# josebeo2016/SCL-Deepfake-audio-detection

Measured on AMD Instinct MI355X. Metric: train-step utterances/sec (64000-sample clips), higher is better.
Workload: dtype bf16

## Files before the change

### scl-deepfake-audio-detection_amd/csrc/gemm_w8.hip

```cpp
#include "gemm_common.h"
#include "gemm_w8_epi.h"

using namespace sclg;

__device__ unsigned long long scl_gemm_stamps[4096 * 8];

namespace {

__device__ __forceinline__ void w8_stamp(const GemmK& d, int slot, int lane, int wave) {
    if ((d.flags & SCL_GEMM_STAMPS) && wave == 0 && lane == 0 && blockIdx.x < 4096 && blockIdx.z == 0) {
        scl_gemm_stamps[blockIdx.x * 8 + 2 * slot] = __builtin_amdgcn_s_memrealtime();
        scl_gemm_stamps[blockIdx.x * 8 + 2 * slot + 1] = __builtin_amdgcn_s_memtime();
    }
}

constexpr int W8_BN = 256;
constexpr int W8_OPB = 2 * TILE_BYTES;
constexpr int W8_NA = 3, W8_NB = 2;
constexpr int W8_LDS = (W8_NA + W8_NB) * W8_OPB;

struct W8K {
    __amdgpu_buffer_rsrc_t rsrc;
    unsigned voff[4];
    __device__ __forceinline__ void init(const OpK& o, const char* base, int row0, int rowlimit, int lane, int wave) {
// ... 330 lines not shown
#define W8S_B_ISSUE(j) if ((j) < 2) { lb.issue1(tB, wave, soffB, live2b, 2 * (j)); lb.issue1(tB, wave, soffB, live2b, 2 * (j) + 1); }
#define W8S_Q_SECOND(j, R0, R1)                                                                                              \
        RD::template go<R0, R1, false>(fa0, fb0, a_nxt, tBn, ab, nbk, 0, lane);                                              \
        __builtin_amdgcn_sched_barrier(0);                                                                                   \
        _Pragma("unroll") for (int i = 0; i < RBW; ++i)                                                                      \
            acc[i][j] = __builtin_amdgcn_mfma_f32_16x16x32_bf16(fb1[j], fa1[i], acc[i][j], 0, 0, 0);                         \
        __builtin_amdgcn_sched_barrier(0);                                                                                   \
        W8S_B_ISSUE(j)                                                                                                       \
        __builtin_amdgcn_sched_barrier(0);
        W8S_Q_SECOND(0, 0, RQ0) W8S_Q_SECOND(1, RQ0, RQ1) W8S_Q_SECOND(2, RQ1, RQ2) W8S_Q_SECOND(3, RQ2, NRD)
#undef W8S_Q_SECOND
#undef W8S_B_ISSUE
        char* t = a_cur; a_cur = a_nxt; a_nxt = a_fill; a_fill = t;
    }
    asm volatile("s_waitcnt vmcnt(0)" ::: "memory");
    asm volatile("s_waitcnt lgkmcnt(0)" ::: "memory");
    __builtin_amdgcn_s_barrier();
    w8_stamp(d, 2, lane, wave);
    {
        const long long cbase = z1 * d.c_bs1 + z2 * d.c_bs2 + (long long)ksplit * d.c_split_stride;
        const float* bias = (d.flags & SCL_GEMM_HAS_BIAS) ? d.bias + z2 * d.bias_bs2 : nullptr;
        char* wlds = smem + wave * 16384;
        char* wextra = smem + 8 * 16384 + wave * 4096;
        float* cs0 = d.colsum ? d.colsum + ((long long)(m0 / d.tile_m) * 4 + (wave >> 2) * 2) * d.N : nullptr;
        if constexpr (RBW >= 4) {
            f32x4 (&alo)[4][4] = *reinterpret_cast<f32x4 (*)[4][4]>(&acc[0]);
            w8_epilogue_pass<4, ((RBW < 8 && !AT) ? 0x1E : 0)>(d, alo, 4, wlds, wextra, m0 + ab * 16, n0 + wc * 64, mlimit, cbase, bias, lane, cs0);
        } else {
            f32x4 lo[4][4];
#pragma unroll
            for (int i = 0; i < 4; ++i)
#pragma unroll
                for (int j = 0; j < 4; ++j) lo[i][j] = (i < RBW) ? acc[(i < RBW) ? i : 0][j] : f32x4{0.f, 0.f, 0.f, 0.f};
            w8_epilogue_pass<4, ((RBW < 8 && !AT) ? 0x1E : 0)>(d, lo, RBW, wlds, wextra, m0 + ab * 16, n0 + wc * 64, mlimit, cbase, bias, lane, cs0);
        }
        if (RBW > 4) {
            f32x4 hi[4][4];
#pragma unroll
            for (int i = 0; i < 4; ++i)
#pragma unroll
                for (int j = 0; j < 4; ++j) hi[i][j] = (4 + i < RBW) ? acc[(4 + i < RBW) ? 4 + i : 0][j] : f32x4{0.f, 0.f, 0.f, 0.f};
            w8_epilogue_pass<4, ((RBW < 8 && !AT) ? 0x1E : 0)>(d, hi, RBW - 4, wlds, wextra, m0 + (ab + 4) * 16, n0 + wc * 64, mlimit, cbase, bias, lane, cs0 ? cs0 + d.N : nullptr);
        }
    }
    if (d.flags & SCL_GEMM_STAMPS) {
        asm volatile("s_waitcnt vmcnt(0)" ::: "memory");
        w8_stamp(d, 3, lane, wave);
    }
}

template <bool AT, bool BT, int RB0, int RB1, bool SEQ = false>
__device__ __forceinline__ void w8s_tile(const GemmK& d, char* smem, const int bid, const int nblk, const int bz) {
    const int tid = threadIdx.x, lane = tid & 63;
    const int wave = __builtin_amdgcn_readfirstlane(tid >> 6);
    const int wr = wave >> 2, wc = wave & 3;
    w8_stamp(d, 0, lane, wave);
#ifdef SCL_EXPERIMENTS
    if ((d.debug >> 8) && (bid & 1) && bid < 256 && bz == 0) {
        for (int i = 0; i < (d.debug >> 8); ++i) __builtin_amdgcn_s_sleep(127);
    }
#endif
    const int tiles_m = (d.M + d.tile_m - 1) / d.tile_m, tiles_n = (d.N + W8_BN - 1) / W8_BN;
    int tm, tn;
    tile_coords<SEQ>(bid, nblk, tiles_m, tiles_n, tm, tn, d.group_m);
    const int m0 = tm * d.tile_m, n0 = tn * W8_BN;
    const int mlimit = min(d.M, m0 + d.tile_m);
    int z = bz;
    const int ksplit = __builtin_amdgcn_readfirstlane(z % d.splitk); z /= d.splitk;
    const int z1 = __builtin_amdgcn_readfirstlane(z / d.nb2), z2 = z - z1 * d.nb2;
    const int nk_total = d.K / BK;
    const int nk_per = __builtin_amdgcn_readfirstlane((nk_total + d.splitk - 1) / d.splitk);
    const int kt0 = ksplit * nk_per;
    const int nk = max(0, min(nk_per, nk_total - kt0));
    const char* Ab = reinterpret_cast<const char*>(d.A.ptr) + z1 * d.A.bs1 + z2 * d.A.bs2;
    const char* Bb = reinterpret_cast<const char*>(d.B.ptr) + z1 * d.B.bs1 + z2 * d.B.bs2;

    typename W8Sel<AT>::type la;
    typename W8Sel<BT>::type lb;
    la.init(d.A, Ab, m0, mlimit, lane, wave);
    lb.init(d.B, Bb, n0, d.N, lane, wave);
    la.set_batched(false); lb.set_batched(false);
    const unsigned stepA = W8Sel<AT>::type::kstep(d.A), stepB = W8Sel<BT>::type::kstep(d.B);
    unsigned soffA = (unsigned)kt0 * stepA, soffB = (unsigned)kt0 * stepB;
    la.template issue2<0>(smem, wave, soffA, nk > 0); la.template issue2<2>(smem, wave, soffA, nk > 0);
    lb.template issue2<0>(smem + W8_NA * W8_OPB, wave, soffB, nk > 0); lb.template issue2<2>(smem + W8_NA * W8_OPB, wave, soffB, nk > 0);
    soffA += stepA; soffB += stepB;
    la.template issue2<0>(smem + W8_OPB, wave, soffA, nk > 1); la.template issue2<2>(smem + W8_OPB, wave, soffA, nk > 1);
    lb.template issue2<0>(smem + (W8_NA + 1) * W8_OPB, wave, soffB, nk > 1); lb.template issue2<2>(smem + (W8_NA + 1) * W8_OPB, wave, soffB, nk > 1);
    asm volatile("s_waitcnt vmcnt(8)" ::: "memory");
    w8_stamp(d, 1, lane, wave);
    __builtin_amdgcn_s_barrier();
    if (RB0 == RB1) {
        w8s_body<AT, BT, RB0>(d, smem, la, lb, nk, soffA, soffB, wr * RB0, m0, n0, mlimit, z1, z2, ksplit, lane, wave, wc);
    } else if (wr == 0) {
        w8s_body<AT, BT, RB0>(d, smem, la, lb, nk, soffA, soffB, 0, m0, n0, mlimit, z1, z2, ksplit, lane, wave, wc);
    } else {
        w8s_body<AT, BT, RB1>(d, smem, la, lb, nk, soffA, soffB, RB0, m0, n0, mlimit, z1, z2, ksplit, lane, wave, wc);
    }
}

template <bool AT, bool BT, int RB0, int RB1>
__global__ __launch_bounds__(512, 2) void scl_gemm_w8s_kernel(const GemmK d) {
    extern __shared__ __attribute__((aligned(16))) char smem[];
    w8s_tile<AT, BT, RB0, RB1>(d, smem, blockIdx.x, gridDim.x, blockIdx.z);
}

struct GemmGroupK {
    GemmK k[W8_GROUP_MAX];
    int first[W8_GROUP_MAX + 1];
    int tile0[W8_GROUP_MAX];
    int ntiles[W8_GROUP_MAX];
    int n;
    int xcd_major;
};
typedef const __attribute__((address_space(4))) GemmGroupK* W8GArg;
template <bool AT, bool BT, int RB0, int RB1>
__global__ __launch_bounds__(512, 2) void scl_gemm_w8s_group_kernel(const GemmGroupK g) {
    extern __shared__ __attribute__((aligned(16))) char smem[];
    W8GArg gp = (W8GArg)__builtin_amdgcn_kernarg_segment_ptr();
    const int total = g.first[W8_GROUP_MAX];
    const int x = blockIdx.x & 7, idx = blockIdx.x >> 3, q = total >> 3, r = total & 7;
#ifdef SCL_EXPERIMENTS
    const int pos = (g.xcd_major ? ((x < r ? x * (q + 1) : r * (q + 1) + (x - r) * q) + idx) : (int)blockIdx.x);
#else
    const int pos = (x < r ? x * (q + 1) : r * (q + 1) + (x - r) * q) + idx;
#endif
    int mem = 0;
#pragma unroll
    for (int i = 1; i < W8_GROUP_MAX; ++i) mem += (i < g.n && pos >= g.first[i]) ? 1 : 0;
    mem = __builtin_amdgcn_readfirstlane(mem);
    const int t = __builtin_amdgcn_readfirstlane(pos - gp->first[mem] + gp->tile0[mem]);
#ifdef SCL_EXPERIMENTS
    if (!g.xcd_major) { w8s_tile<AT, BT, RB0, RB1, false>(*(const GemmK*)&gp->k[mem], smem, t, gp->ntiles[mem], 0); return; }
#endif
    w8s_tile<AT, BT, RB0, RB1, true>(*(const GemmK*)&gp->k[mem], smem, t, gp->ntiles[mem], 0);
}

typedef const __attribute__((address_space(4))) GemmK* W8KArg;
__device__ __forceinline__ const GemmK* w8p_args(W8KArg p) {
    asm volatile("" : "+s"(p));
    return (const GemmK*)p;
}
__device__ __forceinline__ int w8p_lane() {
    int l = (int)__builtin_amdgcn_mbcnt_hi(~0u, __builtin_amdgcn_mbcnt_lo(~0u, 0u));
    asm volatile("" : "+v"(l));
    return l;
}
constexpr int W8_EPI_KEY = SCL_GEMM_C_F32 | SCL_GEMM_C2_F32 | SCL_GEMM_R_F32 | SCL_GEMM_HAS_BIAS | SCL_GEMM_HAS_C2 | SCL_GEMM_DROPOUT |
                           (0xF << SCL_GEMM_ACT_SHIFT) | (0xF << SCL_GEMM_RMODE_SHIFT) | (0xF << SCL_GEMM_RACT_SHIFT);
inline int w8p_epi_kind(int flags) {
    const int f = flags & W8_EPI_KEY, fb = f & ~SCL_GEMM_HAS_BIAS;
    if (fb == 0) return 1;
    if (f == (SCL_GEMM_HAS_BIAS | SCL_GEMM_HAS_C2 | (5 << SCL_GEMM_ACT_SHIFT))) return 2;
    if (fb == SCL_GEMM_C_F32) return 5;
    return 0;
}

template <bool AT, bool BT, int RBW, int EK>
__device__ __forceinline__ void w8p_body(W8KArg kp, char* smem, const int ab, const int lane, const int wave, const int wc) {
    typedef typename W8Sel<AT>::type LA;
    typedef typename W8Sel<BT>::type LB;
    typedef W8SRead<AT, BT, RBW> RD;
    constexpr int NRD = RBW + 4, OPA = AT ? 2 : 1, OPB = BT ? 2 : 1;
    constexpr int RQ0 = 4, RQ1 = 8, RQ2 = NRD;
    static_assert(RBW >= 6 && RBW <= 8, "w8p_body: 6 to 8 row blocks per wave");
    auto ops_upto = [](int n) constexpr { return (n > 0 ? OPB : 0) + (n > 1 ? (n - 1 < RBW ? n - 1 : RBW) * OPA : 0) + (n > RBW + 1 ? (n - RBW - 1) * OPB : 0); };
    const int nbk = wc * 4;
    char* const bimg = smem + W8_NA * W8_OPB;
    char *a_cur = smem, *a_nxt = smem + W8_OPB, *a_fill = smem + 2 * W8_OPB;
    LA la;
    LB lb;
    la.set_batched(false); lb.set_batched(false);
    int nk, tile_m, Mrows, group_m, tiles_m, tiles_n, m0, n0, mlimit;
    unsigned stepA, stepB;
    int v = blockIdx.x;
    {
        const GemmK* d0 = w8p_args(kp);
        nk = d0->K / BK;
        tile_m = d0->tile_m; Mrows = d0->M; group_m = d0->group_m;
        tiles_m = __builtin_amdgcn_readfirstlane((Mrows + tile_m - 1) / tile_m);
        tiles_n = (d0->N + W8_BN - 1) / W8_BN;
        if (v >= tiles_m * tiles_n) return;
        stepA = LA::kstep(d0->A); stepB = LB::kstep(d0->B);
        int tm, tn;
        tile_coords(v, tiles_m * tiles_n, tiles_m, tiles_n, tm, tn, group_m);
        m0 = tm * tile_m; n0 = tn * W8_BN; mlimit = min(Mrows, m0 + tile_m);
        la.init(d0->A, reinterpret_cast<const char*>(d0->A.ptr), m0, mlimit, lane, wave);
        lb.init(d0->B, reinterpret_cast<const char*>(d0->B.ptr), n0, d0->N, lane, wave);
    }
    const int ntiles = tiles_m * tiles_n, G = gridDim.x;
    la.template issue2<0>(a_cur, wave, 0u, true); la.template issue2<2>(a_cur, wave, 0u, true);
    lb.template issue2<0>(bimg, wave, 0u, true); lb.template issue2<2>(bimg, wave, 0u, true);
    la.template issue2<0>(a_nxt, wave, stepA, true); la.template issue2<2>(a_nxt, wave, stepA, true);
    lb.template issue2<0>(bimg + W8_OPB, wave, stepB, true); lb.template issue2<2>(bimg + W8_OPB, wave, stepB, true);
    asm volatile("s_waitcnt vmcnt(8)" ::: "memory");
    __builtin_amdgcn_s_barrier();
    int bpar = 0;
    unsigned soffA = stepA, soffB = stepB;
    int m0n = 0, n0n = 0, mlimn = 0;
    for (;;) {
        f32x4 acc[RBW][4];
#pragma unroll
        for (int i = 0; i < RBW; ++i)
#pragma unroll
            for (int j = 0; j < 4; ++j) acc[i][j] = f32x4{0.f, 0.f, 0.f, 0.f};
        bf16x8 fa0[RBW], fa1[RBW], fb0[4], fb1[4];
        const bool has_next = v + G < ntiles;
        lds_wait_upto(0);
        __builtin_amdgcn_sched_barrier(0);
        RD::template go<0, NRD, true>(fa0, fb0, a_cur, bimg + bpar * W8_OPB, ab, nbk, 0, lane);
        for (int kt = 0; kt < nk; ++kt) {
            char* tB = bimg + ((kt + bpar) & 1) * W8_OPB;
            const bool live2 = kt + 2 < nk || has_next;
            soffA += stepA; soffB += stepB;
            if (kt + 2 == nk) {
                soffA = 0u; soffB = 0u;
                if (has_next) {
                    int tm, tn;
                    tile_coords(v + G, ntiles, tiles_m, tiles_n, tm, tn, group_m);
                    m0n = tm * tile_m; n0n = tn * W8_BN; mlimn = min(Mrows, m0n + tile_m);
                    const GemmK* dh = w8p_args(kp);
                    const int ln = w8p_lane();
                    la.init(dh->A, reinterpret_cast<const char*>(dh->A.ptr), m0n, mlimn, ln, wave);
                    lb.init(dh->B, reinterpret_cast<const char*>(dh->B.ptr), n0n, dh->N, ln, wave);
                    lds_wait_upto(0);
                    __builtin_amdgcn_sched_barrier(0);
                }
            }
#define W8P_Q_FIRST(j, R0, R1)                                                                                               \
            RD::template go<R0, R1, false>(fa1, fb1, a_cur, tB, ab, nbk, 1, lane);                                           \
            __builtin_amdgcn_sched_barrier(0);                                                                               \
            lds_wait_upto((3 - (j)) * OPB + ops_upto(R1));                                                                   \
            __builtin_amdgcn_sched_barrier(0);                                                                               \
            _Pragma("unroll") for (int i = 0; i < RBW; ++i)                                                                  \
                acc[i][j] = __builtin_amdgcn_mfma_f32_16x16x32_bf16(fb0[j], fa0[i], acc[i][j], 0, 0, 0);                     \
            __builtin_amdgcn_sched_barrier(0);                                                                               \
            la.issue1(a_fill, wave, soffA, live2, j);                                                                        \
            __builtin_amdgcn_sched_barrier(0);
            W8P_Q_FIRST(0, 0, RQ0) W8P_Q_FIRST(1, RQ0, RQ1) W8P_Q_FIRST(2, RQ1, RQ2) W8P_Q_FIRST(3, RQ2, NRD)
#undef W8P_Q_FIRST
            lds_wait_upto(0);
            asm volatile("s_waitcnt vmcnt(4)" ::: "memory");
            __builtin_amdgcn_sched_barrier(0);
            __builtin_amdgcn_s_barrier();
            __builtin_amdgcn_sched_barrier(0);
            const char* tBn = bimg + (((kt + bpar) & 1) ^ 1) * W8_OPB;
#define W8P_B_ISSUE(j) if ((j) < 2) { lb.issue1(tB, wave, soffB, live2, 2 * (j)); lb.issue1(tB, wave, soffB, live2, 2 * (j) + 1); }
#define W8P_Q_SECOND(j, R0, R1)                                                                                              \
            RD::template go<R0, R1, false>(fa0, fb0, a_nxt, tBn, ab, nbk, 0, lane);                                          \
            __builtin_amdgcn_sched_barrier(0);                                                                               \
            _Pragma("unroll") for (int i = 0; i < RBW; ++i)                                                                  \
                acc[i][j] = __builtin_amdgcn_mfma_f32_16x16x32_bf16(fb1[j], fa1[i], acc[i][j], 0, 0, 0);                     \
            __builtin_amdgcn_sched_barrier(0);                                                                               \
            W8P_B_ISSUE(j)                                                                                                   \
            __builtin_amdgcn_sched_barrier(0);
            W8P_Q_SECOND(0, 0, RQ0) W8P_Q_SECOND(1, RQ0, RQ1) W8P_Q_SECOND(2, RQ1, RQ2) W8P_Q_SECOND(3, RQ2, NRD)
#undef W8P_Q_SECOND
#undef W8P_B_ISSUE
            char* t = a_cur; a_cur = a_nxt; a_nxt = a_fill; a_fill = t;
        }
        lds_wait_upto(0);
        __builtin_amdgcn_sched_barrier(0);
        {
            const GemmK& d = *w8p_args(kp);
            const int ln = w8p_lane();
            const float* bias = (EK == 2 || (d.flags & SCL_GEMM_HAS_BIAS)) ? d.bias : nullptr;
            char* wlds = a_fill + wave * 4096;
            float* cs0 = d.colsum ? d.colsum + ((long long)(m0 / tile_m) * 4 + (wave >> 2) * 2) * d.N : nullptr;
            float cs[8];
#pragma unroll
            for (int b = 0; b < RBW; ++b) {
                if (b == 0 || b == 4) {
#pragma unroll
                    for (int j = 0; j < 8; ++j) cs[j] = 0.f;
                }
                f32x4 (&a1)[1][4] = *reinterpret_cast<f32x4 (*)[1][4]>(&acc[b]);
                w8_epilogue_pass_k<1, EK>(d, a1, 1, wlds, wlds, m0 + (ab + b) * 16, n0 + wc * 64, mlimit, 0ll, bias, ln, nullptr, cs, 4096);
                if (cs0 && (b == 3 || b == RBW - 1)) w8_colsum_store(d, cs, cs0 + (b >> 2) * d.N, n0 + wc * 64, ln);
            }
        }
        if (!has_next) break;
        bpar = (bpar + nk) & 1;
        v += G; m0 = m0n; n0 = n0n; mlimit = mlimn;
    }
}

template <bool AT, bool BT, int EK, int RB0, int RB1>
__global__ __launch_bounds__(512, 2) void scl_gemm_persist_w8_kernel(const GemmK d) {
    extern __shared__ __attribute__((aligned(16))) char smem[];
    const int tid = threadIdx.x, lane = tid & 63;
    const int wave = __builtin_amdgcn_readfirstlane(tid >> 6);
    W8KArg kp = (W8KArg)__builtin_amdgcn_kernarg_segment_ptr();
    if (RB0 == RB1) w8p_body<AT, BT, RB0, EK>(kp, smem, (wave >> 2) * RB0, lane, wave, wave & 3);
    else if ((wave >> 2) == 0) w8p_body<AT, BT, RB0, EK>(kp, smem, 0, lane, wave, wave & 3);
    else w8p_body<AT, BT, RB1, EK>(kp, smem, RB0, lane, wave, wave & 3);
}

template <bool AT, bool BT, int EK, int RB0, int RB1>
void w8p_launch_k(const GemmK& k, dim3 grid, hipStream_t s) {
    static bool attr_set = false;
    if (!attr_set) {
        (void)hipFuncSetAttribute((const void*)scl_gemm_persist_w8_kernel<AT, BT, EK, RB0, RB1>, hipFuncAttributeMaxDynamicSharedMemorySize, W8_LDS);
        attr_set = true;
    }
    SCL_LAUNCH((scl_gemm_persist_w8_kernel<AT, BT, EK, RB0, RB1>), grid, dim3(512), W8_LDS, s, k);
}
bool w8p_built(bool bt, int ek, int variant) {
    if (variant == 0) return ek == 1 || ek == 2 || ek == 5;
    return variant == 1 && ((!bt && ek == 5) || (bt && ek == 1));
}
void w8p_launch(const GemmK& k, bool bt, int ek, int variant, dim3 grid, hipStream_t s) {
    if (variant == 1) {
        if (!bt) w8p_launch_k<false, false, 5, 8, 8>(k, grid, s);
        else w8p_launch_k<false, true, 1, 8, 8>(k, grid, s);
    } else if (!bt) {
        if (ek == 1) w8p_launch_k<false, false, 1, 7, 6>(k, grid, s);
        else if (ek == 2) w8p_launch_k<false, false, 2, 7, 6>(k, grid, s);
        else w8p_launch_k<false, false, 5, 7, 6>(k, grid, s);
    } else {
        if (ek == 1) w8p_launch_k<false, true, 1, 7, 6>(k, grid, s);
        else if (ek == 2) w8p_launch_k<false, true, 2, 7, 6>(k, grid, s);
        else w8p_launch_k<false, true, 5, 7, 6>(k, grid, s);
    }
}


template <int RB0, int RB1>
void w8_launch_rb(const GemmK& k, bool at, bool bt, dim3 grid, hipStream_t s, int mode) {
    static bool attr_set = false;
    if (!attr_set) {
        (void)hipFuncSetAttribute((const void*)scl_gemm_w8_kernel<false, false, RB0, RB1>, hipFuncAttributeMaxDynamicSharedMemorySize, W8_LDS);
        (void)hipFuncSetAttribute((const void*)scl_gemm_w8_kernel<false, true, RB0, RB1>, hipFuncAttributeMaxDynamicSharedMemorySize, W8_LDS);
        (void)hipFuncSetAttribute((const void*)scl_gemm_w8_kernel<true, false, RB0, RB1>, hipFuncAttributeMaxDynamicSharedMemorySize, W8_LDS);
        (void)hipFuncSetAttribute((const void*)scl_gemm_w8_kernel<true, true, RB0, RB1>, hipFuncAttributeMaxDynamicSharedMemorySize, W8_LDS);
        (void)hipFuncSetAttribute((const void*)scl_gemm_w8s_kernel<false, false, RB0, RB1>, hipFuncAttributeMaxDynamicSharedMemorySize, W8_LDS);
        (void)hipFuncSetAttribute((const void*)scl_gemm_w8s_kernel<false, true, RB0, RB1>, hipFuncAttributeMaxDynamicSharedMemorySize, W8_LDS);
        (void)hipFuncSetAttribute((const void*)scl_gemm_w8s_kernel<true, false, RB0, RB1>, hipFuncAttributeMaxDynamicSharedMemorySize, W8_LDS);
        (void)hipFuncSetAttribute((const void*)scl_gemm_w8s_kernel<true, true, RB0, RB1>, hipFuncAttributeMaxDynamicSharedMemorySize, W8_LDS);
        attr_set = true;
    }
    const dim3 block(512);
    if (mode == 1) {
        if (!at && !bt) SCL_LAUNCH((scl_gemm_w8s_kernel<false, false, RB0, RB1>), grid, block, W8_LDS, s, k);
        else if (!at && bt) SCL_LAUNCH((scl_gemm_w8s_kernel<false, true, RB0, RB1>), grid, block, W8_LDS, s, k);
        else if (at && !bt) SCL_LAUNCH((scl_gemm_w8s_kernel<true, false, RB0, RB1>), grid, block, W8_LDS, s, k);
        else SCL_LAUNCH((scl_gemm_w8s_kernel<true, true, RB0, RB1>), grid, block, W8_LDS, s, k);
        return;
    }
    if (!at && !bt) SCL_LAUNCH((scl_gemm_w8_kernel<false, false, RB0, RB1>), grid, block, W8_LDS, s, k);
    else if (!at && bt) SCL_LAUNCH((scl_gemm_w8_kernel<false, true, RB0, RB1>), grid, block, W8_LDS, s, k);
    else if (at && !bt) SCL_LAUNCH((scl_gemm_w8_kernel<true, false, RB0, RB1>), grid, block, W8_LDS, s, k);
    else SCL_LAUNCH((scl_gemm_w8_kernel<true, true, RB0, RB1>), grid, block, W8_LDS, s, k);
}

void w8_launch_43(const GemmK& k, bool bt, dim3 grid, hipStream_t s) {
    static bool attr_set = false;
    if (!attr_set) {
        (void)hipFuncSetAttribute((const void*)scl_gemm_w8s_kernel<false, false, 4, 3>, hipFuncAttributeMaxDynamicSharedMemorySize, W8_LDS);
        (void)hipFuncSetAttribute((const void*)scl_gemm_w8s_kernel<false, true, 4, 3>, hipFuncAttributeMaxDynamicSharedMemorySize, W8_LDS);
        attr_set = true;
    }
    if (!bt) SCL_LAUNCH((scl_gemm_w8s_kernel<false, false, 4, 3>), grid, dim3(512), W8_LDS, s, k);
    else SCL_LAUNCH((scl_gemm_w8s_kernel<false, true, 4, 3>), grid, dim3(512), W8_LDS, s, k);
}

}

namespace sclg {

bool scl_gemm_w8_plan(const GemmK& k, bool at, bool bt, const SclGemmDesc& d, long long zdim, int ncu, W8Plan* plan) {
    auto flat_rows = [](const SclOperand& o, long long rows) { return (long long)o.rpb >= rows; };
    const bool tt = at && bt;
    const bool a_ok = at ? (flat_rows(d.A, d.K) || (tt && d.A.rpb >= 1)) : (d.A.cin == 0x7fffffff || d.A.cin == 64 || d.A.cin >= d.K);
    const bool b_ok = bt ? (flat_rows(d.B, d.K) || (tt && d.B.rpb >= 1)) : (d.B.cin == 0x7fffffff || d.B.cin == 64 || d.B.cin >= d.K);
    if (!a_ok || !b_ok || (d.K % BK) != 0) return false;
    const long long tiles_n = (d.N + W8_BN - 1) / W8_BN;
    long long best = -1;
    const char* e43 = getenv("SCL_W8_TILE112");
    const char* epp = getenv("SCL_W8_MODE");
    const bool v43_env = !e43 || atoi(e43) != 0, pingpong_env = epp && *epp && atoi(epp) == 0;
    const bool v43_ok = v43_env && !pingpong_env && !at && zdim == 1 && !d.colsum_part && !(d.flags & SCL_GEMM_STAMPS);
    for (int v = 0; v < (v43_ok ? 3 : 2); ++v) {
        const int bm = v == 0 ? 208 : (v == 1 ? 256 : 112);
        const long long ntm = (d.M + bm - 1) / bm;
        const long long rounds = (ntm * tiles_n * zdim + ncu - 1) / ncu;
        const long long cost = rounds * (bm + W8_BN);
        if (best < 0 || cost < best) {
            best = cost;
            plan->variant = v; plan->tiles_m = (int)ntm; plan->tile_m = (int)((d.M + ntm - 1) / ntm);
            plan->tiles = ntm * tiles_n; plan->cost = cost; plan->ncu = ncu;
        }
    }
    return true;
}

bool scl_gemm_w8_group_member_ok(const GemmK& k, bool at, bool bt, const SclGemmDesc& d) {
    if (!at || !bt || d.nb1 != 1 || d.nb2 != 1 || d.splitk != 1 || (d.K % BK) != 0 || d.K / BK < 3) return false;
    if ((long long)d.A.rpb < (long long)d.K || (long long)d.B.rpb < (long long)d.K) return false;
    if ((d.M % 8) || (d.N % 8) || !k.vec_ok) return false;
    const int plain = SCL_GEMM_A_T | SCL_GEMM_B_T | SCL_GEMM_C_F32;
    return (d.flags & ~(SCL_GEMM_NO_DMA | SCL_GEMM_NO_W8)) == plain && !d.colsum_part;
}

int scl_gemm_w8_group_tiles(const GemmK& k) { return ((k.M + 255) / 256) * ((k.N + W8_BN - 1) / W8_BN); }

int scl_gemm_w8_group_launch(GemmK* ks, int n, const int* tile0, const int* ntile, hipStream_t s) {
    GemmGroupK g = GemmGroupK();
    int total = 0;
    for (int i = 0; i < n; ++i) {
        GemmK& k = ks[i];
        const int ntm = (k.M + 255) / 256;
        k.tile_m = (k.M + ntm - 1) / ntm;
        k.debug = 0;
        g.k[i] = k;
        g.first[i] = total;
        g.ntiles[i] = scl_gemm_w8_group_tiles(k);
        g.tile0[i] = tile0 ? tile0[i] : 0;
        total += ntile ? ntile[i] : g.ntiles[i];
    }
    for (int i = n; i <= W8_GROUP_MAX; ++i) g.first[i] = total;
    g.n = n;
#ifdef SCL_EXPERIMENTS
    static const int xcd_major = [] { const char* e = getenv("SCL_WGRAD_XCD_MAJOR"); return e ? atoi(e) : 1; }();
    g.xcd_major = xcd_major;
#else
    g.xcd_major = 1;
#endif
    static bool attr_set = false;
    if (!attr_set) {
        (void)hipFuncSetAttribute((const void*)scl_gemm_w8s_group_kernel<true, true, 8, 8>, hipFuncAttributeMaxDynamicSharedMemorySize, W8_LDS);
        attr_set = true;
    }
    SCL_LAUNCH((scl_gemm_w8s_group_kernel<true, true, 8, 8>), dim3((unsigned)total), dim3(512), W8_LDS, s, g);
    return 0;
}

static long long w8p_launches = 0;
long long scl_gemm_w8p_launches() { return w8p_launches; }

int scl_gemm_read_stamps(unsigned long long* out, int nblocks) {
    return hipMemcpyFromSymbol(out, HIP_SYMBOL(scl_gemm_stamps), sizeof(unsigned long long) * 8 * (size_t)nblocks) == hipSuccess ? 0 : -1;
}

int scl_gemm_w8_persist_blocks(const GemmK& k, bool at, bool bt, const W8Plan& plan, long long zdim) {
    const char* pe = getenv("SCL_W8_PERSIST");
    const int pv = (pe && *pe) ? atoi(pe) : 1;
    const char* me = getenv("SCL_W8_MODE");
    static const bool epi_generic = [] { const char* e = getenv("SCL_W8_EPI_GENERIC"); return e && atoi(e) != 0; }();
    if (pv <= 0 || (me && *me && atoi(me) != 1) || epi_generic) return 0;
    if (plan.variant > 1 || at || zdim != 1 || k.splitk != 1 || k.K / BK < 3 || (k.flags & SCL_GEMM_STAMPS)) return 0;
    const int ek = w8p_epi_kind(k.flags);
    if (!ek || !w8p_built(bt, ek, plan.variant) || ((unsigned)k.flags & SCL_GEMM_C_SPLIT3) || !k.vec_ok || (k.ldc & 7) || (k.c_rbstride & 7)) return 0;
    if (pv >= 8) return pv > 256 ? 256 : (pv & ~7);
    const long long ncu = plan.ncu >= 8 ? plan.ncu : 256;
    const long long rounds = (plan.tiles + ncu - 1) / ncu;
    long long G = (((plan.tiles + rounds - 1) / rounds) + 7) & ~7ll;
    if (G > (ncu & ~7ll)) G = ncu & ~7ll;
    return (G >= 8 && plan.tiles >= 2 * G) ? (int)G : 0;
}

int scl_gemm_w8_launch(GemmK& k, bool at, bool bt, const W8Plan& plan, long long zdim, hipStream_t s) {
    k.tile_m = plan.tile_m;
    k.debug = 0;
    {
        const long long nb1 = zdim / ((long long)k.nb2 * k.splitk);
        const long long rows = k.M - 1, rpb = (long long)k.c_rpb;
        const long long maxoff = (nb1 - 1) * k.c_bs1 + ((long long)k.nb2 - 1) * k.c_bs2 + (rows / rpb) * k.c_rbstride + (rows % rpb) * k.ldc + k.N;
        if (maxoff * ((k.flags & SCL_GEMM_R_F32) ? 4 : 2) >= 0xFFFFFF00ll) k.debug |= 2;
    }
    const dim3 grid((unsigned)plan.tiles, 1, (unsigned)zdim);
    const char* me = getenv("SCL_W8_MODE");
    int mode = (me && *me) ? atoi(me) : 1;
    if (at && bt) {
        if ((long long)k.A.rpb < (long long)k.K) { k.debug |= 4; mode = 0; }
        if ((long long)k.B.rpb < (long long)k.K) { k.debug |= 8; mode = 0; }
    }
    {
        static const bool epi_generic = [] { const char* e = getenv("SCL_W8_EPI_GENERIC"); return e && atoi(e) != 0; }();
        if (epi_generic) k.debug |= 16;
    }
    dim3 g = grid;
#ifdef SCL_EXPERIMENTS
    {
        const char* sg = getenv("SCL_W8_STAGGER");
        const int stg = sg ? atoi(sg) : 0;
        if (stg > 0 && plan.tiles > 256 && zdim == 1) k.debug |= (stg & 0xFF) << 8;
    }
#endif
    if (mode == 1) {
        const int G = scl_gemm_w8_persist_blocks(k, at, bt, plan, zdim);
        if (G > 0) {
            ++w8p_launches;
            w8p_launch(k, bt, w8p_epi_kind(k.flags), plan.variant, dim3((unsigned)G, 1, 1), s);
            return 0;
        }
    }
    if (plan.variant == 2) w8_launch_43(k, bt, g, s);
    else if (plan.variant == 0) w8_launch_rb<7, 6>(k, at, bt, g, s, mode);
    else w8_launch_rb<8, 8>(k, at, bt, g, s, mode);
    return 0;
}

}
```

### scl-deepfake-audio-detection_amd/csrc/gemm_w8_epi.h

```cpp
#pragma once
#include "gemm_common.h"

namespace sclg {

template <int NMT, int EK>
static __device__ __forceinline__ void w8_epilogue_pass_k(const GemmK& d, f32x4 (&acc)[NMT][4], int nmt, char* wlds, char* wextra, int mbase, int nbase,
                                                   int mlimit, long long cbase, const float* bias, int lane, float* csum_row,
                                                   float* cs_carry, const int blk_stride) {
#pragma clang fp contract(off)
    const int flags = d.flags;
    constexpr bool KN = EK != 0;
    const bool c_f32 = KN ? (EK == 4 || EK == 5) : bool(flags & SCL_GEMM_C_F32);
    const bool c2_f32 = KN ? false : bool(flags & SCL_GEMM_C2_F32);
    const bool r_f32 = KN ? (EK == 4) : bool(flags & SCL_GEMM_R_F32);
    const bool has_bias = EK == 2 ? true : (EK == 3 ? false : bool(flags & SCL_GEMM_HAS_BIAS));
    const bool has_c2 = KN ? (EK == 2) : bool(flags & SCL_GEMM_HAS_C2);
    const bool drop = KN ? false : bool(flags & SCL_GEMM_DROPOUT);
    const int act = KN ? (EK == 2 ? 5 : 0) : ((flags >> SCL_GEMM_ACT_SHIFT) & 0xF);
    const int rmode = KN ? (EK == 3 ? 2 : (EK == 4 ? 1 : 0)) : ((flags >> SCL_GEMM_RMODE_SHIFT) & 0xF);
    const int ract = KN ? (EK == 3 ? 4 : 0) : ((flags >> SCL_GEMM_RACT_SHIFT) & 0xF);
    const int g = lane >> 4, lc = lane & 15;
    const int c = lane & 7, rsub = lane >> 3;
    const int col = nbase + 8 * c;
    const bool colv = d.vec_ok && col + 8 <= d.N;
// ... 41 lines not shown
    }
    const char* rstage = wextra;
    for (int i = 0; i < 2 * nmt; ++i) {
        const bool issue = r_dma && (r_f32 ? (i == 0 || i == 2 || i == 4) : (i & 3) == 0);
        if (issue) {
            if (r_f32 && i == 4) asm volatile("s_waitcnt lgkmcnt(0)" ::: "memory");
            char* dst = i == 0 ? wextra : r_issue(i);
            asm volatile("s_waitcnt vmcnt(0)" ::: "memory");
            rstage = dst - (r_f32 ? i * 2048 : i * 1024);
        }
        const int r = 8 * i + rsub;
        const char* wrow = wlds + (r >> 4) * blk_stride + (r & 15) * 256;
        const f32x4 lo = *reinterpret_cast<const f32x4*>(wrow + (((2 * c) ^ (r & 15)) << 4));
        const f32x4 hi = *reinterpret_cast<const f32x4*>(wrow + (((2 * c + 1) ^ (r & 15)) << 4));
        const int row = mbase + r;
        if (row >= mlimit) continue;
        const unsigned q = udiv_magic((unsigned)row, d.c_magic, d.c_shift);
        const long long off = cbase + (long long)q * d.c_rbstride + (long long)((unsigned)row - q * d.c_rpb) * d.ldc + col;
        float v[8] = {d.alpha * lo[0], d.alpha * lo[1], d.alpha * lo[2], d.alpha * lo[3], d.alpha * hi[0], d.alpha * hi[1], d.alpha * hi[2], d.alpha * hi[3]};
        if (colv) {
            if (has_bias) {
#pragma unroll
                for (int j = 0; j < 8; ++j) v[j] += bb[j];
            }
            float w[8] = {v[0], v[1], v[2], v[3], v[4], v[5], v[6], v[7]};
            if (act == 5) {
#pragma unroll
                for (int j = 0; j < 8; j += 2) gelu_both2(v[j], v[j + 1], w[j], w[j + 1]);
            }
            if (has_c2) {
                if (c2_f32) {
                    float* p = reinterpret_cast<float*>(d.C2) + off;
                    *reinterpret_cast<float4*>(p) = make_float4(w[0], w[1], w[2], w[3]);
                    *reinterpret_cast<float4*>(p + 4) = make_float4(w[4], w[5], w[6], w[7]);
                } else {
                    bf16_t* p = reinterpret_cast<bf16_t*>(d.C2) + off;
                    if (KN || (off & 7) == 0) *reinterpret_cast<uint4*>(p) = make_uint4(pack_bf2(w[0], w[1]), pack_bf2(w[2], w[3]), pack_bf2(w[4], w[5]), pack_bf2(w[6], w[7]));
                    else { *reinterpret_cast<uint2*>(p) = make_uint2(pack_bf2(w[0], w[1]), pack_bf2(w[2], w[3])); *reinterpret_cast<uint2*>(p + 4) = make_uint2(pack_bf2(w[4], w[5]), pack_bf2(w[6], w[7])); }
                }
            }
            if (act == 5) {
            } else if (act == 1) {
#pragma unroll
                for (int j = 0; j < 8; j += 2) gelu2(v[j], v[j + 1]);
            } else if (act) {
#pragma unroll
                for (int j = 0; j < 8; ++j) v[j] = act_f(act, v[j]);
            }
            float rr[8] = {0.f, 0.f, 0.f, 0.f, 0.f, 0.f, 0.f, 0.f};
            if (rmode) {
                if (r_f32) {
                    const float* p = r_dma ? reinterpret_cast<const float*>(rstage + i * 2048 + lane * 16) : reinterpret_cast<const float*>(d.R) + off;
                    const float4 t0 = *reinterpret_cast<const float4*>(p), t1 = *reinterpret_cast<const float4*>(p + (r_dma ? 256 : 4));
                    rr[0] = t0.x; rr[1] = t0.y; rr[2] = t0.z; rr[3] = t0.w; rr[4] = t1.x; rr[5] = t1.y; rr[6] = t1.z; rr[7] = t1.w;
                } else {
                    const bf16_t* p = reinterpret_cast<const bf16_t*>(d.R) + off;
                    uint2 t0, t1;
                    if (r_dma) { const uint4 t = *reinterpret_cast<const uint4*>(rstage + i * 1024 + lane * 16); t0 = make_uint2(t.x, t.y); t1 = make_uint2(t.z, t.w); }
                    else if (KN || (off & 7) == 0) { const uint4 t = *reinterpret_cast<const uint4*>(p); t0 = make_uint2(t.x, t.y); t1 = make_uint2(t.z, t.w); }
                    else { t0 = *reinterpret_cast<const uint2*>(p); t1 = *reinterpret_cast<const uint2*>(p + 4); }
                    rr[0] = __uint_as_float(t0.x << 16); rr[1] = __uint_as_float(t0.x & 0xFFFF0000u);
                    rr[2] = __uint_as_float(t0.y << 16); rr[3] = __uint_as_float(t0.y & 0xFFFF0000u);
                    rr[4] = __uint_as_float(t1.x << 16); rr[5] = __uint_as_float(t1.x & 0xFFFF0000u);
                    rr[6] = __uint_as_float(t1.y << 16); rr[7] = __uint_as_float(t1.y & 0xFFFF0000u);
                }
            }
            if (rmode == 2 && ract == 1) {
#pragma unroll
                for (int j = 0; j < 8; j += 2) { gelu_grad2(rr[j], rr[j + 1]); v[j] *= rr[j]; v[j + 1] *= rr[j + 1]; }
            } else if (rmode == 2 && ract == 4) {
#pragma unroll
                for (int j = 0; j < 8; ++j) v[j] *= rr[j];
            } else if (rmode == 2) {
#pragma unroll
                for (int j = 0; j < 8; ++j) v[j] *= act_grad_f(ract, rr[j]);
            }
            if (drop) {
#pragma unroll
                for (int j = 0; j < 8; ++j) v[j] *= dropout_scale(d.drop_seed, (uint64_t)(off + j), d.drop_p);
            }
            if (rmode == 1) {
#pragma unroll
                for (int j = 0; j < 8; ++j) v[j] += rr[j];
            }
            if (csum_row || cs_carry) {
#pragma unroll
                for (int j = 0; j < 8; ++j) cs[j] += v[j];
            }
            if (c_f32) {
                float* p = reinterpret_cast<float*>(d.C) + off;
                *reinterpret_cast<float4*>(p) = make_float4(v[0], v[1], v[2], v[3]);
                *reinterpret_cast<float4*>(p + 4) = make_float4(v[4], v[5], v[6], v[7]);
            } else if (!KN && ((unsigned)flags & SCL_GEMM_C_SPLIT3)) {
                bf16_t* p = reinterpret_cast<bf16_t*>(d.C) + off;
                const uint4 h = make_uint4(pack_bf2(v[0], v[1]), pack_bf2(v[2], v[3]), pack_bf2(v[4], v[5]), pack_bf2(v[6], v[7]));
                const unsigned hw[4] = {h.x, h.y, h.z, h.w};
                float l8[8];
#pragma unroll
                for (int j = 0; j < 4; ++j) {
                    l8[2 * j] = v[2 * j] - __uint_as_float(hw[j] << 16);
                    l8[2 * j + 1] = v[2 * j + 1] - __uint_as_float(hw[j] & 0xFFFF0000u);
                }
                *reinterpret_cast<uint4*>(p) = h;
                *reinterpret_cast<uint4*>(p + d.N) = h;
                *reinterpret_cast<uint4*>(p + 2 * (long long)d.N) = make_uint4(pack_bf2(l8[0], l8[1]), pack_bf2(l8[2], l8[3]), pack_bf2(l8[4], l8[5]), pack_bf2(l8[6], l8[7]));
            } else {
                bf16_t* p = reinterpret_cast<bf16_t*>(d.C) + off;
                if (KN || (off & 7) == 0) *reinterpret_cast<uint4*>(p) = make_uint4(pack_bf2(v[0], v[1]), pack_bf2(v[2], v[3]), pack_bf2(v[4], v[5]), pack_bf2(v[6], v[7]));
                else { *reinterpret_cast<uint2*>(p) = make_uint2(pack_bf2(v[0], v[1]), pack_bf2(v[2], v[3])); *reinterpret_cast<uint2*>(p + 4) = make_uint2(pack_bf2(v[4], v[5]), pack_bf2(v[6], v[7])); }
            }
        } else {
#pragma unroll
            for (int j = 0; j < 8; ++j) epi_scalar(ea, v[j], off + j, col + j, bias);
        }
    }
    if (cs_carry) {
#pragma unroll
        for (int j = 0; j < 8; ++j) cs_carry[j] = cs[j];
    } else if (csum_row) {
#pragma unroll
        for (int j = 0; j < 8; ++j) {
            cs[j] += __shfl_xor(cs[j], 8, 64);
            cs[j] += __shfl_xor(cs[j], 16, 64);
            cs[j] += __shfl_xor(cs[j], 32, 64);
        }
        if (lane < 8 && colv) {
            *reinterpret_cast<float4*>(csum_row + col) = make_float4(cs[0], cs[1], cs[2], cs[3]);
            *reinterpret_cast<float4*>(csum_row + col + 4) = make_float4(cs[4], cs[5], cs[6], cs[7]);
        }
    }
}


template <int NMT, int SPEC = 0x1E>
static __device__ __forceinline__ void w8_epilogue_pass(const GemmK& d, f32x4 (&acc)[NMT][4], int nmt, char* wlds, char* wextra, int mbase, int nbase,
                                                 int mlimit, long long cbase, const float* bias, int lane, float* csum_row = nullptr,
                                                 float* cs_carry = nullptr, const int blk_stride = 4096) {
    constexpr int KEY = SCL_GEMM_C_F32 | SCL_GEMM_C2_F32 | SCL_GEMM_R_F32 | SCL_GEMM_HAS_BIAS | SCL_GEMM_HAS_C2 | SCL_GEMM_DROPOUT |
                        (0xF << SCL_GEMM_ACT_SHIFT) | (0xF << SCL_GEMM_RMODE_SHIFT) | (0xF << SCL_GEMM_RACT_SHIFT);
    const int f = d.flags & KEY, fb = f & ~SCL_GEMM_HAS_BIAS;
    if (SPEC != 0 && !(d.debug & 16) && !((unsigned)d.flags & SCL_GEMM_C_SPLIT3) && d.vec_ok && !(d.ldc & 7) && !(d.c_rbstride & 7) && !(cbase & 7)) {
        if ((SPEC & 2) && fb == 0) return w8_epilogue_pass_k<NMT, 1>(d, acc, nmt, wlds, wextra, mbase, nbase, mlimit, cbase, bias, lane, csum_row, cs_carry, blk_stride);
        if ((SPEC & 4) && f == (SCL_GEMM_HAS_BIAS | SCL_GEMM_HAS_C2 | (5 << SCL_GEMM_ACT_SHIFT)))
            return w8_epilogue_pass_k<NMT, 2>(d, acc, nmt, wlds, wextra, mbase, nbase, mlimit, cbase, bias, lane, csum_row, cs_carry, blk_stride);
        if ((SPEC & 8) && f == ((2 << SCL_GEMM_RMODE_SHIFT) | (4 << SCL_GEMM_RACT_SHIFT)))
            return w8_epilogue_pass_k<NMT, 3>(d, acc, nmt, wlds, wextra, mbase, nbase, mlimit, cbase, bias, lane, csum_row, cs_carry, blk_stride);
        if ((SPEC & 16) && fb == (SCL_GEMM_C_F32 | SCL_GEMM_R_F32 | (1 << SCL_GEMM_RMODE_SHIFT)))
            return w8_epilogue_pass_k<NMT, 4>(d, acc, nmt, wlds, wextra, mbase, nbase, mlimit, cbase, bias, lane, csum_row, cs_carry, blk_stride);
        if ((SPEC & 32) && fb == SCL_GEMM_C_F32) return w8_epilogue_pass_k<NMT, 5>(d, acc, nmt, wlds, wextra, mbase, nbase, mlimit, cbase, bias, lane, csum_row, cs_carry, blk_stride);
    }
    w8_epilogue_pass_k<NMT, 0>(d, acc, nmt, wlds, wextra, mbase, nbase, mlimit, cbase, bias, lane, csum_row, cs_carry, blk_stride);
}

static __device__ __forceinline__ void w8_colsum_store(const GemmK& d, float (&cs)[8], float* csum_row, int nbase, int lane) {
    const int col = nbase + 8 * (lane & 7);
#pragma unroll
    for (int j = 0; j < 8; ++j) {
        cs[j] += __shfl_xor(cs[j], 8, 64);
        cs[j] += __shfl_xor(cs[j], 16, 64);
        cs[j] += __shfl_xor(cs[j], 32, 64);
    }
    if (lane < 8 && d.vec_ok && col + 8 <= d.N) {
        *reinterpret_cast<float4*>(csum_row + col) = make_float4(cs[0], cs[1], cs[2], cs[3]);
        *reinterpret_cast<float4*>(csum_row + col + 4) = make_float4(cs[4], cs[5], cs[6], cs[7]);
    }
}

}
```

Baseline: 1638.

## Add persistent w8 GEMM path with prefetched residual-multiply epilogue

Extends the persistent w8 GEMM kernel to handle the epilogue kind that multiplies the result by a bf16 residual tensor R (rmode 2, ract 4) with column sums, which previously fell back to a non-persistent kernel. All residual loads for a wave's row blocks are issued up front as raw buffer loads and then awaited with explicit vmcnt counts, so their latency overlaps the LDS transpose and store work. The path is limited to aligned R whose extent fits 32-bit buffer offsets, and it depends on hand-written inline asm wait counts being correct.

```diff
diff --git a/scl-deepfake-audio-detection_amd/csrc/gemm_w8.hip b/scl-deepfake-audio-detection_amd/csrc/gemm_w8.hip
--- a/scl-deepfake-audio-detection_amd/csrc/gemm_w8.hip
+++ b/scl-deepfake-audio-detection_amd/csrc/gemm_w8.hip
@@ -506,6 +506,7 @@
     const int f = flags & W8_EPI_KEY, fb = f & ~SCL_GEMM_HAS_BIAS;
     if (fb == 0) return 1;
     if (f == (SCL_GEMM_HAS_BIAS | SCL_GEMM_HAS_C2 | (5 << SCL_GEMM_ACT_SHIFT))) return 2;
+    if (f == ((2 << SCL_GEMM_RMODE_SHIFT) | (4 << SCL_GEMM_RACT_SHIFT))) return 3;
     if (fb == SCL_GEMM_C_F32) return 5;
     return 0;
 }
@@ -622,15 +623,33 @@
             char* wlds = a_fill + wave * 4096;
             float* cs0 = d.colsum ? d.colsum + ((long long)(m0 / tile_m) * 4 + (wave >> 2) * 2) * d.N : nullptr;
             float cs[8];
-#pragma unroll
-            for (int b = 0; b < RBW; ++b) {
-                if (b == 0 || b == 4) {
-#pragma unroll
-                    for (int j = 0; j < 8; ++j) cs[j] = 0.f;
+            if constexpr (EK == 3) {
+                w8_u32x4 rq[2 * RBW];
+                const w8_u32x4 rs = w8_rsrc_words(d.R);
+                const __amdgpu_buffer_rsrc_t c_rsrc = make_rsrc(reinterpret_cast<const char*>(d.C));
+#pragma unroll
+                for (int b = 0; b < RBW; ++b) w8_xr_request(d, rq[2 * b], rq[2 * b + 1], rs, m0 + (ab + b) * 16, n0 + wc * 64, mlimit, ln, b == 0);
+                __builtin_amdgcn_sched_barrier(0);
+#pragma unroll
+                for (int b = 0; b < RBW; ++b) {
+                    if (b == 0 || b == 4) {
+#pragma unroll
+                        for (int j = 0; j < 8; ++j) cs[j] = 0.f;
+                    }
+                    w8_epilogue_pass_xr<2 * RBW - 2>(d, acc[b], wlds, m0 + (ab + b) * 16, n0 + wc * 64, mlimit, ln, rq[2 * b], rq[2 * b + 1], c_rsrc, cs);
+                    if (cs0 && (b == 3 || b == RBW - 1)) w8_colsum_store(d, cs, cs0 + (b >> 2) * d.N, n0 + wc * 64, ln);
                 }
-                f32x4 (&a1)[1][4] = *reinterpret_cast<f32x4 (*)[1][4]>(&acc[b]);
-                w8_epilogue_pass_k<1, EK>(d, a1, 1, wlds, wlds, m0 + (ab + b) * 16, n0 + wc * 64, mlimit, 0ll, bias, ln, nullptr, cs, 4096);
-                if (cs0 && (b == 3 || b == RBW - 1)) w8_colsum_store(d, cs, cs0 + (b >> 2) * d.N, n0 + wc * 64, ln);
+            } else {
+#pragma unroll
+                for (int b = 0; b < RBW; ++b) {
+                    if (b == 0 || b == 4) {
+#pragma unroll
+                        for (int j = 0; j < 8; ++j) cs[j] = 0.f;
+                    }
+                    f32x4 (&a1)[1][4] = *reinterpret_cast<f32x4 (*)[1][4]>(&acc[b]);
+                    w8_epilogue_pass_k<1, EK>(d, a1, 1, wlds, wlds, m0 + (ab + b) * 16, n0 + wc * 64, mlimit, 0ll, bias, ln, nullptr, cs, 4096);
+                    if (cs0 && (b == 3 || b == RBW - 1)) w8_colsum_store(d, cs, cs0 + (b >> 2) * d.N, n0 + wc * 64, ln);
+                }
             }
         }
         if (!has_next) break;
@@ -650,6 +669,15 @@
     else w8p_body<AT, BT, RB1, EK>(kp, smem, RB0, lane, wave, wave & 3);
 }
 
+__global__ __launch_bounds__(512, 2) void scl_gemm_persist_w8r_kernel(const GemmK d) {
+    extern __shared__ __attribute__((aligned(16))) char smem[];
+    const int tid = threadIdx.x, lane = tid & 63;
+    const int wave = __builtin_amdgcn_readfirstlane(tid >> 6);
+    W8KArg kp = (W8KArg)__builtin_amdgcn_kernarg_segment_ptr();
+    if ((wave >> 2) == 0) w8p_body<false, true, 7, 3>(kp, smem, 0, lane, wave, wave & 3);
+    else w8p_body<false, true, 6, 3>(kp, smem, 7, lane, wave, wave & 3);
+}
+
 template <bool AT, bool BT, int EK, int RB0, int RB1>
 void w8p_launch_k(const GemmK& k, dim3 grid, hipStream_t s) {
     static bool attr_set = false;
@@ -659,12 +687,22 @@
     }
     SCL_LAUNCH((scl_gemm_persist_w8_kernel<AT, BT, EK, RB0, RB1>), grid, dim3(512), W8_LDS, s, k);
 }
+void w8r_launch(const GemmK& k, dim3 grid, hipStream_t s) {
+    static bool attr_set = false;
+    if (!attr_set) {
+        (void)hipFuncSetAttribute((const void*)scl_gemm_persist_w8r_kernel, hipFuncAttributeMaxDynamicSharedMemorySize, W8_LDS);
+        attr_set = true;
+    }
+    SCL_LAUNCH(scl_gemm_persist_w8r_kernel, grid, dim3(512), W8_LDS, s, k);
+}
 bool w8p_built(bool bt, int ek, int variant) {
-    if (variant == 0) return ek == 1 || ek == 2 || ek == 5;
+    if (variant == 0) return ek == 1 || ek == 2 || ek == 5 || (ek == 3 && bt);
     return variant == 1 && ((!bt && ek == 5) || (bt && ek == 1));
 }
 void w8p_launch(const GemmK& k, bool bt, int ek, int variant, dim3 grid, hipStream_t s) {
-    if (variant == 1) {
+    if (ek == 3) {
+        w8r_launch(k, grid, s);
+    } else if (variant == 1) {
         if (!bt) w8p_launch_k<false, false, 5, 8, 8>(k, grid, s);
         else w8p_launch_k<false, true, 1, 8, 8>(k, grid, s);
     } else if (!bt) {
@@ -796,6 +834,13 @@
     return hipMemcpyFromSymbol(out, HIP_SYMBOL(scl_gemm_stamps), sizeof(unsigned long long) * 8 * (size_t)nblocks) == hipSuccess ? 0 : -1;
 }
 
+static bool w8_r_extent_wide(const GemmK& k, long long zdim) {
+    const long long nb1 = zdim / ((long long)k.nb2 * k.splitk);
+    const long long rows = k.M - 1, rpb = (long long)k.c_rpb;
+    const long long maxoff = (nb1 - 1) * k.c_bs1 + ((long long)k.nb2 - 1) * k.c_bs2 + (rows / rpb) * k.c_rbstride + (rows % rpb) * k.ldc + k.N;
+    return maxoff * ((k.flags & SCL_GEMM_R_F32) ? 4 : 2) >= 0xFFFFFF00ll;
+}
+
 int scl_gemm_w8_persist_blocks(const GemmK& k, bool at, bool bt, const W8Plan& plan, long long zdim) {
     const char* pe = getenv("SCL_W8_PERSIST");
     const int pv = (pe && *pe) ? atoi(pe) : 1;
@@ -805,6 +850,7 @@
     if (plan.variant > 1 || at || zdim != 1 || k.splitk != 1 || k.K / BK < 3 || (k.flags & SCL_GEMM_STAMPS)) return 0;
     const int ek = w8p_epi_kind(k.flags);
     if (!ek || !w8p_built(bt, ek, plan.variant) || ((unsigned)k.flags & SCL_GEMM_C_SPLIT3) || !k.vec_ok || (k.ldc & 7) || (k.c_rbstride & 7)) return 0;
+    if (ek == 3 && (((unsigned long long)k.R & 15) || w8_r_extent_wide(k, zdim))) return 0;
     if (pv >= 8) return pv > 256 ? 256 : (pv & ~7);
     const long long ncu = plan.ncu >= 8 ? plan.ncu : 256;
     const long long rounds = (plan.tiles + ncu - 1) / ncu;
@@ -816,12 +862,7 @@
 int scl_gemm_w8_launch(GemmK& k, bool at, bool bt, const W8Plan& plan, long long zdim, hipStream_t s) {
     k.tile_m = plan.tile_m;
     k.debug = 0;
-    {
-        const long long nb1 = zdim / ((long long)k.nb2 * k.splitk);
-        const long long rows = k.M - 1, rpb = (long long)k.c_rpb;
-        const long long maxoff = (nb1 - 1) * k.c_bs1 + ((long long)k.nb2 - 1) * k.c_bs2 + (rows / rpb) * k.c_rbstride + (rows % rpb) * k.ldc + k.N;
-        if (maxoff * ((k.flags & SCL_GEMM_R_F32) ? 4 : 2) >= 0xFFFFFF00ll) k.debug |= 2;
-    }
+    if (w8_r_extent_wide(k, zdim)) k.debug |= 2;
     const dim3 grid((unsigned)plan.tiles, 1, (unsigned)zdim);
     const char* me = getenv("SCL_W8_MODE");
     int mode = (me && *me) ? atoi(me) : 1;
diff --git a/scl-deepfake-audio-detection_amd/csrc/gemm_w8_epi.h b/scl-deepfake-audio-detection_amd/csrc/gemm_w8_epi.h
--- a/scl-deepfake-audio-detection_amd/csrc/gemm_w8_epi.h
+++ b/scl-deepfake-audio-detection_amd/csrc/gemm_w8_epi.h
@@ -217,6 +217,70 @@
     w8_epilogue_pass_k<NMT, 0>(d, acc, nmt, wlds, wextra, mbase, nbase, mlimit, cbase, bias, lane, csum_row, cs_carry, blk_stride);
 }
 
+typedef unsigned w8_u32x4 __attribute__((ext_vector_type(4)));
+
+static __device__ __forceinline__ w8_u32x4 w8_rsrc_words(const void* base) {
+    const unsigned long long b = (unsigned long long)base;
+    return w8_u32x4{(unsigned)__builtin_amdgcn_readfirstlane((unsigned)b), (unsigned)__builtin_amdgcn_readfirstlane((unsigned)(b >> 32)) & 0xFFFFu, 0xFFFFFFFFu, 0x00020000u};
+}
+
+static __device__ __forceinline__ unsigned w8_xr_offset(const GemmK& d, int row, int mlimit, int col, bool colv) {
+    const unsigned q = udiv_magic((unsigned)row, d.c_magic, d.c_shift);
+    const long long o = (long long)q * d.c_rbstride + (long long)((unsigned)row - q * d.c_rpb) * d.ldc + col;
+    return (row < mlimit && colv) ? (unsigned)(o << 1) : OOB;
+}
+
+static __device__ __forceinline__ void w8_xr_request(const GemmK& d, w8_u32x4& r0, w8_u32x4& r1, const w8_u32x4 rs, int mbase, int nbase, int mlimit, int lane, bool first) {
+    const int c = lane & 7, rsub = lane >> 3, col = nbase + 8 * c;
+    const bool colv = d.vec_ok && col + 8 <= d.N;
+    const unsigned o0 = w8_xr_offset(d, mbase + rsub, mlimit, col, colv), o1 = w8_xr_offset(d, mbase + 8 + rsub, mlimit, col, colv);
+    if (first) asm volatile("s_nop 4\n\tbuffer_load_dwordx4 %0, %1, %2, 0 offen" : "=v"(r0) : "v"(o0), "s"(rs) : "memory");
+    else asm volatile("buffer_load_dwordx4 %0, %1, %2, 0 offen" : "=v"(r0) : "v"(o0), "s"(rs) : "memory");
+    asm volatile("buffer_load_dwordx4 %0, %1, %2, 0 offen" : "=v"(r1) : "v"(o1), "s"(rs) : "memory");
+}
+
+template <int PENDING>
+static __device__ __forceinline__ void w8_epilogue_pass_xr(const GemmK& d, f32x4 (&acc)[4], char* wlds, int mbase, int nbase, int mlimit, int lane,
+                                                           w8_u32x4& r0, w8_u32x4& r1, __amdgpu_buffer_rsrc_t c_rsrc, float (&cs)[8]) {
+#pragma clang fp contract(off)
+    static_assert(PENDING >= 0 && PENDING < 63, "w8_epilogue_pass_xr: a six-bit counter");
+    const int g = lane >> 4, lc = lane & 15;
+    const int c = lane & 7, rsub = lane >> 3;
+    const int col = nbase + 8 * c;
+    const bool colv = d.vec_ok && col + 8 <= d.N;
+#pragma unroll
+    for (int nt = 0; nt < 4; ++nt) *reinterpret_cast<f32x4*>(wlds + lc * 256 + (((nt * 4 + g) ^ lc) << 4)) = acc[nt];
+    const EpiArgs ea = {d.C, d.C2, d.R, d.N, d.flags, d.drop_seed, d.drop_p};
+#pragma unroll
+    for (int i = 0; i < 2; ++i) {
+        const int r = 8 * i + rsub;
+        const char* wrow = wlds + r * 256;
+        const f32x4 lo = *reinterpret_cast<const f32x4*>(wrow + (((2 * c) ^ r) << 4));
+        const f32x4 hi = *reinterpret_cast<const f32x4*>(wrow + (((2 * c + 1) ^ r) << 4));
+        const int row = mbase + r;
+        const bool rowv = row < mlimit;
+        const unsigned q = udiv_magic((unsigned)row, d.c_magic, d.c_shift);
+        const long long off = (long long)q * d.c_rbstride + (long long)((unsigned)row - q * d.c_rpb) * d.ldc + col;
+        float v[8] = {d.alpha * lo[0], d.alpha * lo[1], d.alpha * lo[2], d.alpha * lo[3], d.alpha * hi[0], d.alpha * hi[1], d.alpha * hi[2], d.alpha * hi[3]};
+        if (i == 0) asm volatile("s_waitcnt vmcnt(%2)" : "+v"(r0), "+v"(r1) : "n"(PENDING) : "memory");
+        const w8_u32x4 t = i ? r1 : r0;
+        const float rr[8] = {__uint_as_float(t.x << 16), __uint_as_float(t.x & 0xFFFF0000u), __uint_as_float(t.y << 16), __uint_as_float(t.y & 0xFFFF0000u),
+                             __uint_as_float(t.z << 16), __uint_as_float(t.z & 0xFFFF0000u), __uint_as_float(t.w << 16), __uint_as_float(t.w & 0xFFFF0000u)};
+#pragma unroll
+        for (int j = 0; j < 8; ++j) v[j] *= rr[j];
+        if (rowv && colv) {
+#pragma unroll
+            for (int j = 0; j < 8; ++j) cs[j] += v[j];
+        }
+        const w8_u32x4 pk = {pack_bf2(v[0], v[1]), pack_bf2(v[2], v[3]), pack_bf2(v[4], v[5]), pack_bf2(v[6], v[7])};
+        __builtin_amdgcn_raw_buffer_store_b128(pk, c_rsrc, (rowv && colv) ? (unsigned)(off << 1) : OOB, 0, 0);
+        if (rowv && !colv) {
+#pragma unroll
+            for (int j = 0; j < 8; ++j) epi_scalar(ea, d.alpha * (j < 4 ? lo[j] : hi[j - 4]), off + j, col + j, nullptr);
+        }
+    }
+}
+
 static __device__ __forceinline__ void w8_colsum_store(const GemmK& d, float (&cs)[8], float* csum_row, int nbase, int lane) {
     const int col = nbase + 8 * (lane & 7);
 #pragma unroll
```

Result: no change. 1652, median of 6 (+0.8%).
